# TheShinning/gps-sdr-sim

Hardware: AMD Instinct MI355X
Metric: IQ MSamples/s (and × real-time) at 2.6 MS/s, 12 sats, -b 16; 1/2/4/8 GPU (higher is better)
Workload: dtype int64 phases + f16 x f16 -> f32 MFMA accumulate (exact integer sums)

## Files before the change

### gps-sdr-sim_amd/csrc/common/gss_lin.h

```cpp
#ifndef GSS_LIN_H
#define GSS_LIN_H

#include <stdint.h>

#ifndef GSS_LIN_CH
#define GSS_LIN_CH     16
#endif
#define GSS_LIN_CHUNK  (64 * GSS_LIN_CH)
#define GSS_LIN_SEG    4096

#if defined(__HIPCC__)
#define GSS_LIN_FN static __host__ __device__ inline
#else
#define GSS_LIN_FN static inline
#endif

#define GSS_LIN_CSH    26

GSS_LIN_FN uint32_t gss_lin_dx(uint64_t xs) { return (uint32_t)((xs * 64u + (1ull << 31)) >> 32); }
GSS_LIN_FN uint32_t gss_lin_dz(uint64_t zs)
{
    return (uint32_t)((zs * 64u + (1ull << (GSS_LIN_CSH - 1))) >> GSS_LIN_CSH);
}
GSS_LIN_FN uint64_t gss_lin_xa(uint64_t xs)
// ... 50 lines not shown
}

typedef struct {
    uint64_t x;
    uint64_t z;
    int32_t g01;
    int32_t pos1;
    uint32_t npatch;
    uint32_t pad;
} gss_lin_row;
typedef struct {
    uint64_t xs, zs;
    uint64_t d;
    uint32_t dq;
    uint32_t tab;
} gss_lin_chan;

GSS_LIN_FN uint64_t gss_lin_mulhi(uint64_t a, uint64_t b)
{
#if defined(__HIP_DEVICE_COMPILE__)
    return __umul64hi(a, b);
#else
    return (uint64_t)(((unsigned __int128)a * b) >> 64);
#endif
}

GSS_LIN_FN uint64_t gss_lin_row_x(uint64_t x0, uint64_t xs, uint64_t n0)
{
    return x0 + n0 * xs + gss_lin_xa(xs);
}
GSS_LIN_FN uint64_t gss_lin_row_z(uint64_t z0, uint64_t zs, uint64_t n0)
{
    const uint64_t lo = z0 + n0 * zs;
    const uint64_t hi = gss_lin_mulhi(n0, zs) + (lo < z0 ? 1u : 0u);
    const uint32_t e0 = gss_lin_e0((hi << 14) | (lo >> 50));
    return (((uint64_t)e0 << 50) | (lo & ((1ull << 50) - 1))) + gss_lin_za(zs);
}
GSS_LIN_FN void gss_lin_row_gain(gss_lin_row *r, const int32_t *gpos, const int32_t *gval, int ngc,
                                 int32_t n0)
{
    int32_t g0 = gval[0], gn = 0, pn = INT32_MAX;
    for (int i = 1; i < ngc; i++) {
        const int32_t p = gpos[i], v = gval[i];
        g0 = p <= n0 ? v : g0;
    }
    for (int i = ngc - 1; i >= 1; i--) {
        const int32_t p = gpos[i], v = gval[i];
        gn = p > n0 ? v : gn;
        pn = p > n0 ? p : pn;
    }
    const int more = pn < n0 + GSS_LIN_SEG;
    const int32_t g1 = more ? gn : g0;
    r->g01 = (int32_t)(((uint32_t)g0 & 0xFFFFu) | ((uint32_t)g1 << 16));
    r->pos1 = more ? pn : INT32_MAX;
}
GSS_LIN_FN uint32_t gss_lin_row_npatch(const int32_t *ppos, int np, int32_t n0)
{
    uint32_t n = 0;
    for (int j = 0; j < np; j++)
        n += ppos[j] >= n0 && ppos[j] < n0 + GSS_LIN_SEG;
    return n;
}
GSS_LIN_FN gss_lin_row gss_lin_row_at(uint64_t x0, uint64_t xs, uint64_t z0, uint64_t zs,
                                      const int32_t *gpos, const int32_t *gval, int ngc,
                                      const int32_t *ppos, int np, int32_t n0)
{
    gss_lin_row r;
    r.x = gss_lin_row_x(x0, xs, (uint64_t)n0);
    r.z = gss_lin_row_z(z0, zs, (uint64_t)n0);
    gss_lin_row_gain(&r, gpos, gval, ngc, n0);
    r.npatch = gss_lin_row_npatch(ppos, np, n0);
    r.pad = 0;
    return r;
}
GSS_LIN_FN gss_lin_chan gss_lin_chan_of(uint64_t xs, uint64_t zs, uint32_t ca_tbl)
{
    gss_lin_chan c;
    c.xs = xs;
    c.zs = zs;
    c.d = ((uint64_t)gss_lin_dx(xs) << 32) | gss_lin_dz(zs);
    c.dq = (uint32_t)((zs * 64u) >> 46);
    c.tab = ca_tbl;
    return c;
}

typedef struct {
    int cell, chip;
} gss_lin_kc;

GSS_LIN_FN gss_lin_kc gss_lin_kernel_at(uint64_t x0, uint64_t xs, uint64_t z0, uint64_t zs,
                                         int64_t p)
{
    const int64_t c = p & ~(int64_t)(GSS_LIN_CHUNK - 1);
    const int64_t l = p & 63, s = (p - c) >> 6;
    const uint64_t lane = gss_lin_lane(xs, zs, (uint32_t)l);
    const int64_t n0 = p & ~(int64_t)(GSS_LIN_SEG - 1);
    const unsigned __int128 zn = (unsigned __int128)z0 + (unsigned __int128)(uint64_t)n0 * zs;
    const int64_t chips = (int64_t)(zn >> 50), e0 = gss_lin_e0((uint64_t)chips);
    const __int128 z = (__int128)z0 + (__int128)c * (__int128)zs -
                      (__int128)(chips - e0) * ((__int128)1 << 50);
    const unsigned __int128 zk = (unsigned __int128)((z + (int64_t)gss_lin_za(zs)) >> GSS_LIN_CSH);
    const uint64_t za = (uint64_t)(uint32_t)zk + (uint32_t)lane;
    const uint64_t zw = (uint64_t)(uint32_t)za + (uint64_t)s * gss_lin_dz(zs);
    const unsigned __int128 kz = zk + (uint32_t)lane + (unsigned __int128)(uint64_t)s *
                                 gss_lin_dz(zs);
    const uint32_t xb = (uint32_t)((x0 + (uint64_t)c * xs + gss_lin_xa(xs)) >> 32);
    const uint32_t xk = xb + (uint32_t)(lane >> 32) + (uint32_t)(za >> 32) +
                        (uint32_t)s * gss_lin_dx(xs) + (uint32_t)(zw >> 32);
    gss_lin_kc r;
    r.cell = (int)(xk >> 23);
    r.chip = (int)((uint64_t)(kz >> 24) % 1023u);
    return r;
}

#endif
```

### gps-sdr-sim_amd/csrc/hip/gss_synth.hip

```cpp
#include <hip/hip_runtime.h>
#include <stdint.h>
#include <stdlib.h>
#include <string.h>
#include "gpssim_amd.h"
#include "gss_dev.h"
#include "../common/gss_phase.h"
#include "../common/gss_lin.h"

#define SYNTH_THREADS  256
#define SYNTH_WAVES    (SYNTH_THREADS / 64)
#define ANCHOR_THREADS 64
#define CHUNK_BYTES    128
#define CHUNK_PIECES   (CHUNK_BYTES / 16)
#define LUT_N          1024

__global__ __launch_bounds__(ANCHOR_THREADS) void gss_anchor_kernel(
    const gss_chan_blk_t *__restrict__ blk, const int32_t *__restrict__ nch,
    const double *__restrict__ carr_ck, int nblk, int nchp, int n_per_blk, int nseg, int nsegp,
    int seg_r, double *__restrict__ seg_carr, double *__restrict__ seg_code,
    uint32_t *__restrict__ seg_cnt, double *__restrict__ carr_end,
    const int32_t *__restrict__ blist)
{
    const int nsub = carr_ck ? GSS_NCK : 1;
    const int nbw = (nblk + ANCHOR_THREADS - 1) / ANCHOR_THREADS;
// ... 298 lines not shown
                uint32_t ai = 64, aq = 64;
#pragma unroll
                for (int k = 0; k < NCH; k++) {
                    const int cv = (int)((uint32_t)e[k] << 10) >> 10;
                    const int sv = (e[k] - cv) >> 22;
                    ai += (uint32_t)g[k] * (uint32_t)cv;
                    aq += (uint32_t)g[k] * (uint32_t)sv;
                }
                acc_i = (int)ai;
                acc_q = (int)aq;
            }
#pragma unroll
            for (int k = 0; k < NCH; k++) {
                carr[k] = gss_carr_wrap(carr[k] + cs[k]);
                C[k] = C[k] + ks[k];
            }
            int i16 = (int)(int16_t)(acc_i >> 7);
            int q16 = (int)(int16_t)(acc_q >> 7);
            if (FMT == 16) {
                mine[sidx] = (uint32_t)(uint16_t)i16 | ((uint32_t)(uint16_t)q16 << 16);
            } else if (FMT == 8) {
                ((uint16_t *)mine)[sidx] = (uint16_t)((uint32_t)(uint8_t)(int8_t)(i16 >> 4) |
                                           ((uint32_t)(uint8_t)(int8_t)(q16 >> 4) << 8));
            } else {
                bits = (bits << 2) | ((uint32_t)(i16 > 0) << 1) | (uint32_t)(q16 > 0);
                if ((sidx & 15) == 15) {
                    int nb = nsamp - (sidx & ~15);
                    uint32_t w32 = nb >= 16 ? bits : nb > 0 ? (bits >> 2 * (16 - nb)) << 2 * (16 - nb) : 0u;
                    mine[sidx >> 4] = __builtin_bswap32(w32);
                    bits = 0;
                }
            }
        }
        if (last_seg && full && (ch + 1) * SPC == len) {
#pragma unroll
            for (int k = 0; k < NCH; k++) {
                const uint32_t c = s_st[k][tid];
                bad |= (C[k] >= GSS_CA_SEQ_LEN_D && c == (19u | (29u << 5) | (59u << 10))) ? 1 : 0;
            }
        }
        const bool any_full = __any(full);
        if (any_full) {
            wave_sync_lds();
            for (int i = 0; i < CHUNK_PIECES; i++) {
                int src = (64 / CHUNK_PIECES) * i + lane / CHUNK_PIECES, piece = lane % CHUNK_PIECES;
                int src_full = __shfl(full ? 1 : 0, src);
                if (src_full) {
                    uint8_t *sdst = dst + (ptrdiff_t)(src - lane) * ((ptrdiff_t)seg_r * BPS4 / 4) +
                                    (size_t)ch * CHUNK_BYTES + piece * 16;
                    const uint32_t *sp = stg + src * (CHUNK_BYTES / 4) + piece * 4;
                    store16(sdst, make_uint4(sp[0], sp[1], sp[2], sp[3]));
                }
            }
            wave_sync_lds();
        }
        if (!full && nsamp > 0) {
            int nbytes = nsamp * BPS4 / 4;
            uint8_t *bp = dst + (size_t)ch * CHUNK_BYTES;
            const uint8_t *sp = (const uint8_t *)mine;
            for (int i = 0; i < nbytes; i++)
                bp[i] = sp[i];
        }
    }
    if (bad && status)
        atomicOr(status, bad);
}

#define LIN_THREADS 256
#define LIN_WAVES   (LIN_THREADS / 64)
#define LIN_STEPS   (GSS_LIN_SEG / 64)
#define LIN_CH      GSS_LIN_CH
#define CBW_PRE     2
#define CBW_CHIPS   3072
#define CAB_W       ((CBW_CHIPS + 96) / 32)
static_assert(LIN_STEPS % LIN_CH == 0 && (LIN_CH & (LIN_CH - 1)) == 0, "whole chunks");
#define LIN_SW_SGPRS 68
typedef _Float16 lin_half4 __attribute__((ext_vector_type(4)));
typedef _Float16 lin_half8 __attribute__((ext_vector_type(8)));
typedef float lin_f4 __attribute__((ext_vector_type(4)));
#define LIN_GS    2
#define LIN_MAGF  (12582912.0f + 64.0f * LIN_GS)
#define LIN_MAGB  0x4B400000u

struct alignas(16) lin_ct {
    uint64_t B;
    uint64_t D;
    int32_t g;
    int32_t gd;
    int32_t pos1;
    uint32_t flags;
    uint32_t q0, dq, tab;
    uint32_t wa;
    uint32_t na, nb;
    uint32_t wn;
    uint32_t g2;
    uint32_t A[5][2];
};
static_assert(offsetof(lin_ct, A) % 8 == 0, "lin_ct.A: 8-byte reads");

typedef gss_lin_row lin_seg;
typedef gss_lin_chan lin_chan;
static_assert(sizeof(lin_seg) == 32 && sizeof(lin_chan) == 32, "two 16-byte LDS reads each");

__global__ void gss_cab_kernel(const uint32_t *__restrict__ ca_bits, int n_ca,
                               uint32_t *__restrict__ cab)
{
    const int i = blockIdx.x * blockDim.x + threadIdx.x;
    if (i >= n_ca * CAB_W)
        return;
    const int row = i / CAB_W, j0 = (i - row * CAB_W) * 32 - 32;
    const uint32_t *cb = ca_bits + (size_t)row * GSS_CA_WORDS;
    uint32_t w = 0;
    for (int q = 0; q < 32; q++) {
        const int e = j0 + q, chip = ((e % GSS_CA_LEN) + GSS_CA_LEN) % GSS_CA_LEN;
        w |= (((cb[chip >> 5] >> (chip & 31)) & 1u) ^ 1u) << q;
    }
    cab[i] = w;
}

__global__ void gss_tw16_kernel(const uint32_t *__restrict__ cab, int n_ca, uint32_t w,
                                uint32_t *__restrict__ tw)
{
    const int i = blockIdx.x * blockDim.x + threadIdx.x;
    if (i >= n_ca * GSS_LIN_TWE * LIN_CH)
        return;
    const int row = i / (GSS_LIN_TWE * LIN_CH), r = i - row * (GSS_LIN_TWE * LIN_CH);
    const int E = r / LIN_CH, st = r % LIN_CH;
    const uint32_t j = min((uint32_t)(E + (int)(((uint32_t)st * w) >> 4) - GSS_LIN_CBW_PRE + 32),
                           (uint32_t)(32 * CAB_W - 64));
    const uint32_t *c = cab + (size_t)row * CAB_W;
    const uint32_t lin = __builtin_amdgcn_alignbit(c[(j >> 5) + 1], c[j >> 5], j & 31);
    tw[i] = __builtin_amdgcn_alignbit(lin, lin, (32u - j) & 31u);
}

struct lin_wsrc {
    const uint32_t *W;
};

__device__ __forceinline__ void lin_wissue(const lin_wsrc &w, uint32_t (&ws)[LIN_CH])
{
#pragma unroll
    for (int s = 0; s < LIN_CH; s++)
        ws[s] = w.W[s];
}

__device__ __forceinline__ void lin_wfence(const uint32_t (&ws)[LIN_CH])
{
    static_assert(LIN_CH == 16, "the fence below names 16 windows");
    asm volatile("" :: "s"(ws[0]), "s"(ws[1]), "s"(ws[2]), "s"(ws[3]), "s"(ws[4]), "s"(ws[5]),
                 "s"(ws[6]), "s"(ws[7]), "s"(ws[8]), "s"(ws[9]), "s"(ws[10]), "s"(ws[11]),
                 "s"(ws[12]), "s"(ws[13]), "s"(ws[14]), "s"(ws[15]));
}

__device__ __forceinline__ lin_wsrc lin_wsrc_of(const lin_ct &t, const uint32_t *__restrict__ tw)
{
    const uint32_t off = __builtin_amdgcn_readfirstlane(t.wa);
    return lin_wsrc{(const uint32_t *)__builtin_assume_aligned(
        (const char *)tw + off, 64)};
}

#define LIN_SW_CLOBB "s84", "s85", "s86", "s87", "s88", "s89", "s90", "s91", "s92", "s93", "s94", \
                     "s95", "s96", "s97", "s98", "s99"
#define LIN_SW_CLOBA "s68", "s69", "s70", "s71", "s72", "s73", "s74", "s75", "s76", "s77", "s78", \
                     "s79", "s80", "s81", "s82", "s83"
#pragma clang diagnostic push
#pragma clang diagnostic ignored "-Winline-asm"
__device__ __forceinline__ void lin_sw_load(const uint32_t *__restrict__ tw, uint32_t off)
{
    const uint32_t *p = (const uint32_t *)((const char *)tw +
                                           (uint32_t)__builtin_amdgcn_readfirstlane(off));
    asm volatile("s_load_dwordx16 s[84:99], %0, 0x0" : : "s"(p) : LIN_SW_CLOBB);
}
__device__ __forceinline__ void lin_sw_load2(const uint32_t *__restrict__ tw, uint32_t off_a,
                                             uint32_t off_b)
{
    const uint32_t *pa = (const uint32_t *)((const char *)tw +
                                            (uint32_t)__builtin_amdgcn_readfirstlane(off_a));
    const uint32_t *pb = (const uint32_t *)((const char *)tw +
                                            (uint32_t)__builtin_amdgcn_readfirstlane(off_b));
    asm volatile("s_load_dwordx16 s[68:83], %0, 0x0\n\ts_load_dwordx16 s[84:99], %1, 0x0"
                 : : "s"(pa), "s"(pb) : LIN_SW_CLOBA, LIN_SW_CLOBB);
}
#pragma clang diagnostic pop
#define LIN_SW_TAKE(BUF, W)                                                                       \
    asm volatile("s_waitcnt lgkmcnt(0)\n\t"                                                      \
                 "s_mov_b64 %0, s[" #BUF "+0:" #BUF "+1]\n\ts_mov_b64 %1, s[" #BUF "+2:" #BUF "+3]\n\t" \
                 "s_mov_b64 %2, s[" #BUF "+4:" #BUF "+5]\n\ts_mov_b64 %3, s[" #BUF "+6:" #BUF "+7]\n\t" \
                 "s_mov_b64 %4, s[" #BUF "+8:" #BUF "+9]\n\ts_mov_b64 %5, s[" #BUF "+10:" #BUF "+11]\n\t" \
                 "s_mov_b64 %6, s[" #BUF "+12:" #BUF "+13]\n\ts_mov_b64 %7, s[" #BUF "+14:" #BUF "+15]" \
                 : "=s"(W[0]), "=s"(W[1]), "=s"(W[2]), "=s"(W[3]), "=s"(W[4]), "=s"(W[5]),      \
                   "=s"(W[6]), "=s"(W[7]))
__device__ __forceinline__ void lin_sw_split(const uint64_t (&w)[8], uint32_t (&ws)[LIN_CH])
{
    static_assert(LIN_CH == 16, "16 windows");
#pragma unroll
    for (int i = 0; i < 8; i++) {
        ws[2 * i] = (uint32_t)w[i];
        ws[2 * i + 1] = (uint32_t)(w[i] >> 32);
    }
}
__device__ __forceinline__ void lin_sw_take(uint32_t (&ws)[LIN_CH])
{
    uint64_t w[8];
    LIN_SW_TAKE(84, w);
    lin_sw_split(w, ws);
}
__device__ __forceinline__ void lin_sw_take_a(uint32_t (&ws)[LIN_CH])
{
    uint64_t w[8];
    LIN_SW_TAKE(68, w);
    lin_sw_split(w, ws);
}

template <bool LANE_GAIN, bool FIRST = false>
__device__ __forceinline__ void lin_channel_chunk_m(lin_f4 (&cq)[LIN_CH / 2], lin_f4 c0, uint64_t P,
                                                    uint64_t D, lin_wsrc W, uint32_t M,
                                                    lin_half4 A, int pos1, int p0,
                                                    const int32_t *__restrict__ s_lut)
{
    uint32_t e0 = 0;
    uint32_t sw[LIN_CH];
    lin_wissue(W, sw);
    lin_wfence(sw);
#pragma unroll
    for (int s = 0; s < LIN_CH; s++) {
        const uint32_t ws = sw[s];
        uint32_t t;
        asm("v_lshrrev_b32_sdwa %0, %1, %2 dst_sel:DWORD dst_unused:UNUSED_PAD src0_sel:BYTE_3 "
            "src1_sel:DWORD" : "=v"(t) : "v"((uint32_t)P), "s"(ws));
        const uint32_t a = __builtin_amdgcn_alignbit(t, (uint32_t)(P >> 32), 21) & M;
        uint32_t e = *(const uint32_t *)((const char *)s_lut + a);
        if (LANE_GAIN)
            e = p0 + s * 64 >= pos1 ? e : 0u;
        if (s & 1) {
            const uint2 bb = make_uint2(e0, e);
            cq[s / 2] = __builtin_amdgcn_mfma_f32_4x4x4f16(A, __builtin_bit_cast(lin_half4, bb),
                                                          FIRST ? c0 : cq[s / 2], 0, 0, 0);
        } else {
            e0 = e;
        }
        P += D;
    }
}

__device__ __forceinline__ void lin_sw_steps(lin_f4 (&cq)[LIN_CH / 2], const lin_ct &t, int k,
                                             int lane, const uint64_t *s_lane, uint32_t M,
                                             const int32_t *__restrict__ s_lut,
                                             const uint32_t (&ws)[LIN_CH])
{
    uint64_t P = s_lane[k * 64 + lane] + t.B;
    const uint64_t D = t.D;
    const lin_half4 A = __builtin_bit_cast(lin_half4, *(const uint2 *)t.A[lane & 3]);
    uint32_t e0 = 0;
#pragma unroll
    for (int s = 0; s < LIN_CH; s++) {
        uint32_t tt;
        asm("v_lshrrev_b32_sdwa %0, %1, %2 dst_sel:DWORD dst_unused:UNUSED_PAD src0_sel:BYTE_3 "
            "src1_sel:DWORD" : "=v"(tt) : "v"((uint32_t)P), "s"(ws[s]));
        const uint32_t a = __builtin_amdgcn_alignbit(tt, (uint32_t)(P >> 32), 21) & M;
        const uint32_t e = *(const uint32_t *)((const char *)s_lut + a);
        if (s & 1) {
            const uint2 bb = make_uint2(e0, e);
            cq[s / 2] = __builtin_amdgcn_mfma_f32_4x4x4f16(A, __builtin_bit_cast(lin_half4, bb),
                                                          cq[s / 2], 0, 0, 0);
        } else {
            e0 = e;
        }
        P += D;
    }
}

__device__ __forceinline__ uint32_t lin_pair_cls(int lane)
{
    const int q = lane >> 4, r = lane & 3;
    return ((lane & 15) >> 2) == q ? (uint32_t)r : 4u;
}

template <bool FIRST>
__device__ __forceinline__ void lin_sw_pair(lin_f4 (&cq)[LIN_CH / 2], lin_f4 c0, const lin_ct *T, int k0,
                                            int nc, int lane, const uint64_t *s_lane, uint32_t M,
                                            const int32_t *__restrict__ s_lut,
                                            const uint32_t *__restrict__ tw, uint32_t cls,
                                            bool more)
{
    const lin_ct &ta = T[k0], &tb = T[k0 + 1];
    uint64_t Pa = s_lane[k0 * 64 + lane] + ta.B, Pb = s_lane[(k0 + 1) * 64 + lane] + tb.B;
    const uint64_t Da = ta.D, Db = tb.D;
    const uint2 ga = *(const uint2 *)ta.A[cls], gb = *(const uint2 *)tb.A[cls];
    const lin_half8 A = __builtin_bit_cast(lin_half8, make_uint4(ga.x, ga.y, gb.x, gb.y));
    uint32_t na = ta.na, nb = ta.nb;
    asm volatile("" : "+v"(na), "+v"(nb));
    uint32_t wsa[LIN_CH], wsb[LIN_CH];
    lin_sw_take_a(wsa);
    lin_sw_take(wsb);
    if (k0 + 2 < nc || more)
        lin_sw_load2(tw, na, nb);
    uint32_t ea0 = 0, eb0 = 0;
#pragma unroll
    for (int s = 0; s < LIN_CH; s++) {
        uint32_t ta_, tb_;
        asm("v_lshrrev_b32_sdwa %0, %1, %2 dst_sel:DWORD dst_unused:UNUSED_PAD src0_sel:BYTE_3 "
            "src1_sel:DWORD" : "=v"(ta_) : "v"((uint32_t)Pa), "s"(wsa[s]));
        asm("v_lshrrev_b32_sdwa %0, %1, %2 dst_sel:DWORD dst_unused:UNUSED_PAD src0_sel:BYTE_3 "
            "src1_sel:DWORD" : "=v"(tb_) : "v"((uint32_t)Pb), "s"(wsb[s]));
        const uint32_t aa = __builtin_amdgcn_alignbit(ta_, (uint32_t)(Pa >> 32), 21) & M;
        const uint32_t ab = __builtin_amdgcn_alignbit(tb_, (uint32_t)(Pb >> 32), 21) & M;
        const uint32_t ea = *(const uint32_t *)((const char *)s_lut + aa);
        const uint32_t eb = *(const uint32_t *)((const char *)s_lut + ab);
        if (s & 1) {
            const uint4 bb = make_uint4(ea0, ea, eb0, eb);
            cq[s / 2] = __builtin_amdgcn_mfma_f32_16x16x32_f16(A, __builtin_bit_cast(lin_half8, bb),
                                                              FIRST ? c0 : cq[s / 2], 0, 0, 0);
        } else {
            ea0 = ea;
            eb0 = eb;
        }
        Pa += Da;
        Pb += Db;
    }
}

__device__ __forceinline__ lin_half4 lin_gain_operand(uint32_t gh, int lane)
{
    const uint32_t x = gh << ((lane & 1) * 16);
    const uint2 v = (lane & 2) ? make_uint2(0u, x) : make_uint2(x, 0u);
    return __builtin_bit_cast(lin_half4, v);
}

__host__ __device__ __forceinline__ uint32_t lin_f16_bits(int g)
{
    return (uint32_t)__builtin_bit_cast(uint16_t, (_Float16)(float)g);
}

__device__ __forceinline__ void lin_put(uint32_t *p, uint32_t v)
{
    __builtin_nontemporal_store(v, p);
}

extern "C" __device__ int gss_writelane(int, int, int) __asm("llvm.amdgcn.writelane.i32");

__device__ __forceinline__ uint32_t lin_ib(const lin_f4 (&cq)[LIN_CH / 2], int s)
{
    return __float_as_uint(cq[s / 2][2 * (s & 1)]);
}
__device__ __forceinline__ uint32_t lin_qb(const lin_f4 (&cq)[LIN_CH / 2], int s)
{
    return __float_as_uint(cq[s / 2][2 * (s & 1) + 1]);
}
__device__ __forceinline__ uint32_t lin_w16(const lin_f4 (&cq)[LIN_CH / 2], int s)
{
    const uint32_t pq = __builtin_amdgcn_perm(lin_qb(cq, s), lin_ib(cq, s), 0x06050201u);
    uint32_t r;
    asm("v_pk_add_u16 %0, %1, %2" : "=v"(r) : "v"(pq), "s"(0xC000C000u));
    return r;
}
__device__ __forceinline__ uint32_t lin_w8(const lin_f4 (&cq)[LIN_CH / 2], int s)
{
    constexpr uint32_t sh = 12u;
    uint32_t d = lin_ib(cq, s) >> sh;
    asm("v_lshrrev_b32_sdwa %0, %1, %2 dst_sel:BYTE_1 dst_unused:UNUSED_PRESERVE src0_sel:DWORD "
        "src1_sel:DWORD" : "+v"(d) : "v"(sh), "v"(lin_qb(cq, s)));
    return d;
}
__device__ __forceinline__ bool lin_ipos(const lin_f4 (&cq)[LIN_CH / 2], int s)
{
    return lin_ib(cq, s) >= LIN_MAGB + 128u * LIN_GS;
}
__device__ __forceinline__ bool lin_qpos(const lin_f4 (&cq)[LIN_CH / 2], int s)
{
    return lin_qb(cq, s) >= LIN_MAGB + 128u * LIN_GS;
}

template <int FMT, bool TAIL>
__device__ __forceinline__ void lin_store(const lin_f4 (&acc)[LIN_CH / 2], uint8_t *__restrict__ ob,
                                          int nb0, int lane, int n_per_blk)
{
    static_assert(FMT != 1 || LIN_CH == 16, "-b 1 packing assumes 16-step chunks");
    uint32_t pk[LIN_CH];
    pk[0] = 0;
#pragma unroll
    for (int s = 0; s < LIN_CH; s++) {
        const int nb = nb0 + s * 64, p = nb + lane;
        const bool in = !TAIL || p < n_per_blk;
        if (FMT == 16) {
            pk[s] = lin_w16(acc, s);
        } else if (FMT == 8) {
            const uint32_t v = lin_w8(acc, s);
            if (!TAIL)
                asm volatile("global_store_short %0, %1, %2 offset:%3"
                             : : "v"((uint32_t)lane * 2u), "v"(v),
                               "s"((uint16_t *)ob + nb0 + (s >> 4) * 2048), "i"((s & 15) * 128)
                             : "memory");
            else if (in)
                ((uint16_t *)ob)[p] = (uint16_t)v;
        } else {
            const uint64_t mi = __builtin_amdgcn_ballot_w64(lin_ipos(acc, s));
            const uint64_t mq = __builtin_amdgcn_ballot_w64(lin_qpos(acc, s));
            const uint32_t ilo = (uint32_t)mi, ihi = (uint32_t)(mi >> 32);
            const uint32_t qlo = (uint32_t)mq, qhi = (uint32_t)(mq >> 32);
            pk[0] = (uint32_t)gss_writelane((int)((ilo & 0xFFFFu) | (qlo << 16)), 4 * s, (int)pk[0]);
            pk[0] = (uint32_t)gss_writelane((int)((ilo >> 16) | (qlo & 0xFFFF0000u)), 4 * s + 1, (int)pk[0]);
            pk[0] = (uint32_t)gss_writelane((int)((ihi & 0xFFFFu) | (qhi << 16)), 4 * s + 2, (int)pk[0]);
            pk[0] = (uint32_t)gss_writelane((int)((ihi >> 16) | (qhi & 0xFFFF0000u)), 4 * s + 3, (int)pk[0]);
            (void)in;
        }
    }
    if (FMT == 1) {
        uint32_t vi = pk[0] & 0xFFFFu, vq = pk[0] >> 16;
        vi = (vi | (vi << 8)) & 0x00FF00FFu; vq = (vq | (vq << 8)) & 0x00FF00FFu;
        vi = (vi | (vi << 4)) & 0x0F0F0F0Fu; vq = (vq | (vq << 4)) & 0x0F0F0F0Fu;
        vi = (vi | (vi << 2)) & 0x33333333u; vq = (vq | (vq << 2)) & 0x33333333u;
        vi = (vi | (vi << 1)) & 0x55555555u; vq = (vq | (vq << 1)) & 0x55555555u;
        const uint32_t x = (vi << 1) | vq;
        const uint32_t y = ((x & 0x03030303u) << 6) | ((x & 0x0C0C0C0Cu) << 2) |
                           ((x >> 2) & 0x0C0C0C0Cu) | ((x >> 6) & 0x03030303u);
        uint8_t *dst = ob + nb0 / 4 + 4 * lane;
        const int first = nb0 + 16 * lane;
        const bool whole = !TAIL || first + 16 <= n_per_blk;
        if (whole && ((uintptr_t)(ob + nb0 / 4) & 3u) == 0) {
            lin_put((uint32_t *)dst, y);
        } else {
            for (int b = 0; b < 4; b++)
                if (first + 4 * b < n_per_blk)
                    dst[b] = (uint8_t)(y >> (8 * b));
        }
    }
    if (FMT == 16) {
        __builtin_amdgcn_sched_barrier(0);
        if (!TAIL) {
            uint32_t *base = (uint32_t *)ob + nb0;
            const uint32_t off = (uint32_t)lane * 4u;
#pragma unroll
            for (int s = 0; s < LIN_CH; s++)
                asm volatile("global_store_dword %0, %1, %2 offset:%3 nt"
                             : : "v"(off), "v"(pk[s]), "s"(base + (s >> 4) * 1024),
                               "i"((s & 15) * 256) : "memory");
        } else {
#pragma unroll
            for (int s = 0; s < LIN_CH; s++) {
                const int p = nb0 + s * 64 + lane;
                if (!TAIL || p < n_per_blk)
                    lin_put(((uint32_t *)ob) + p, pk[s]);
            }
        }
    }
}

__device__ __forceinline__ void lin_patch_fix(lin_f4 (&cq)[LIN_CH / 2],
                                              const gss_lin_t *__restrict__ Lk, int nb0, int lane)
{
    for (int j = 0; j < GSS_NPATCH; j++) {
        const int pp = Lk->ppos[j];
        if (pp >= nb0 + 64 * LIN_CH)
            break;
        if (pp < nb0)
            continue;
        const int q = pp - nb0;
        const int64_t d = lane == (q & 63) ? Lk->pdelta[j] : 0;
        const int di = (int)((uint32_t)d << 10) >> 10;
        const float fi = (float)(di * LIN_GS), fq = (float)((int)((d - di) >> 22) * LIN_GS);
        const int sq = __builtin_amdgcn_readfirstlane(q >> 6);
#pragma unroll
        for (int s = 0; s < LIN_CH; s++) {
            const float m = s == sq ? 1.0f : 0.0f;
            cq[s / 2][2 * (s & 1)] = __builtin_fmaf(m, fi, cq[s / 2][2 * (s & 1)]);
            cq[s / 2][2 * (s & 1) + 1] = __builtin_fmaf(m, fq, cq[s / 2][2 * (s & 1) + 1]);
        }
    }
}


#define LIN_MINB 4
template <int FMT>
__global__ __launch_bounds__(LIN_THREADS, LIN_MINB) __attribute__((amdgpu_num_sgpr(LIN_SW_SGPRS)))
void gss_lin_kernel(
    const gss_lin_t *__restrict__ lin, const gss_chan_blk_t *__restrict__ blk,
    const int32_t *__restrict__ nch, const int32_t *__restrict__ fast,
    const uint32_t *__restrict__ cab, const uint32_t *__restrict__ tw,
    const uint4 *__restrict__ lut16, int n_per_blk, int wg_per_blk,
    uint8_t *__restrict__ out, size_t block_bytes)
{
    __shared__ alignas(16) int32_t s_lut[1024];
    __shared__ uint64_t s_lane[GSS_MAXCH * 64];
    __shared__ lin_ct s_ct[LIN_WAVES][GSS_MAXCH];
    __shared__ alignas(16) lin_seg s_seg[LIN_WAVES][GSS_MAXCH];
    __shared__ alignas(16) lin_chan s_chan[GSS_MAXCH];
    const int b = blockIdx.x / wg_per_blk;
    const int w = blockIdx.x - b * wg_per_blk;
    if (!fast[b])
        return;
    const int tid = threadIdx.x, lane = tid & 63;
    const int wave = __builtin_amdgcn_readfirstlane(tid >> 6);
    static_assert(sizeof(s_lut) == LIN_THREADS * sizeof(uint4), "one 16-byte copy per thread");
    const uint4 lutv = lut16[tid];
    const gss_lin_t *L = lin + (size_t)b * GSS_MAXCH;
    const int nc = nch[b];
#pragma unroll
    for (int j = 0; j < GSS_MAXCH / LIN_WAVES; j++) {
        const int k = wave + j * LIN_WAVES;
        if (k < nc)
            s_lane[k * 64 + lane] = gss_lin_lane(L[k].xs, L[k].zs, (uint32_t)lane);
    }
    {
        const int rk = lane & (GSS_MAXCH - 1), rj = lane / GSS_MAXCH;
        static_assert(LIN_WAVES * GSS_MAXCH == 64 && LIN_WAVES == 4, "one row per lane, 4 parts");
        const int rn0 = (w * LIN_WAVES + rj) * (64 * LIN_STEPS);
        if (rk < nc && rn0 < n_per_blk) {
            const gss_lin_t *Lk = L + rk;
            lin_seg &r = s_seg[rj][rk];
            if (wave == 0) {
                r.x = gss_lin_row_x(Lk->x0, Lk->xs, (uint64_t)rn0);
                r.z = gss_lin_row_z(Lk->z0, Lk->zs, (uint64_t)rn0);
            } else if (wave == 1) {
                gss_lin_row g;
                gss_lin_row_gain(&g, Lk->gpos, Lk->gval, GSS_NGC, rn0);
                r.g01 = g.g01;
                r.pos1 = g.pos1;
            } else if (wave == 2) {
                r.npatch = gss_lin_row_npatch(Lk->ppos, GSS_NPATCH, rn0);
                r.pad = 0;
            } else if (rj == 0) {
                s_chan[rk] = gss_lin_chan_of(Lk->xs, Lk->zs,
                                             (uint32_t)blk[(size_t)b * GSS_MAXCH + rk].ca_tbl);
            }
        }
    }
    ((uint4 *)s_lut)[tid] = lutv;
    (void)cab;
    __syncthreads();
    uint32_t M = 0xFFCu;
    asm volatile("" : "+v"(M));
    const uint32_t cls = lin_pair_cls(lane);
    lin_f4 c0 = lin_f4{LIN_MAGF, LIN_MAGF, LIN_MAGF, LIN_MAGF};
    asm volatile("" : "+v"(c0));
    const int sg = w * LIN_WAVES + wave;
    const int n0 = sg * (64 * LIN_STEPS);
    if (n0 >= n_per_blk)
        return;
    lin_ct *T = s_ct[wave];
    uint8_t *ob = out + (size_t)b * block_bytes;
    bool sw_ahead = false;
    uint64_t xb = 0, zb = 0, xs10 = 0, zs10 = 0;
    int32_t pos1 = INT32_MAX;
    uint32_t pflag = 0, gh0 = 0, gh1 = 0;
    uint32_t trow = 0, wa_next = 0;
    int g_after = -1;
    if (lane < nc) {
        const lin_chan ck = s_chan[lane];
        const lin_seg sk = s_seg[wave][lane];
        xb = sk.x;
        zb = sk.z;
        xs10 = ck.xs << 10;
        zs10 = ck.zs << 10;
        static_assert(64 * LIN_CH == 1024, "one chunk = 2^10 samples");
        pos1 = sk.pos1;
        pflag = sk.npatch != 0 ? 2u : 0u;
        const int g0 = (int)(int16_t)(sk.g01 & 0xFFFF), g1 = sk.g01 >> 16;
        gh0 = lin_f16_bits(g0 * LIN_GS);
        gh1 = lin_f16_bits(g1 * LIN_GS);
        lin_ct &t = T[lane];
        t.D = ck.d;
        t.gd = g1 - g0;
        t.pos1 = sk.pos1;
        t.dq = ck.dq;
        t.tab = ck.tab;
        t.A[4][0] = 0;
        t.A[4][1] = 0;
        trow = ck.tab * GSS_LIN_TWE;
        wa_next = (trow + min((uint32_t)(zb >> 50), (uint32_t)(GSS_LIN_TWE - 1))) *
                  (uint32_t)(LIN_CH * sizeof(uint32_t));
    }

    const int nc_blk = nc;
    for (int c = 0; c < LIN_STEPS / LIN_CH; c++) {
        int nc = nc_blk;
        asm volatile("" : "+s"(nc));
        const int nb0 = n0 + c * (64 * LIN_CH);
        if (nb0 >= n_per_blk)
            break;
        const bool after = pos1 <= nb0;
        const bool chg = pos1 < nb0 + 64 * LIN_CH;
        const uint32_t my_flags = (chg && !after ? 1u : 0u) | pflag;
        const uint64_t zn = zb + zs10;
        const uint32_t my_wa = wa_next;
        const uint32_t my_wn = (trow + min((uint32_t)(zn >> 50), (uint32_t)(GSS_LIN_TWE - 1))) *
                               (uint32_t)(LIN_CH * sizeof(uint32_t));
        if (lane < nc) {
            lin_ct &t = T[lane];
            t.B = (xb & ~0xFFFFFFFFull) | (uint32_t)(zb >> GSS_LIN_CSH);
            t.flags = my_flags;
            t.wa = my_wa;
            t.wn = my_wn;
            if ((int)after != g_after) {
                g_after = (int)after;
                const uint32_t gh = after ? gh1 : gh0;
                t.A[0][0] = gh;         t.A[0][1] = 0;
                t.A[1][0] = gh << 16;   t.A[1][1] = 0;
                t.A[2][0] = 0;          t.A[2][1] = gh;
                t.A[3][0] = 0;          t.A[3][1] = gh << 16;
                t.g2 = gh | (gh << 16);
            }
        }
        wa_next = my_wn;
        xb += xs10;
        zb = zn;
        const uint32_t wa0 = (uint32_t)__builtin_amdgcn_readlane((int)my_wa, 0);
        const uint32_t wa1r = (uint32_t)__builtin_amdgcn_readlane((int)my_wa, 1);
        const uint32_t wn0 = (uint32_t)__builtin_amdgcn_readlane((int)my_wn, 0);
        const uint32_t wn1r = (uint32_t)__builtin_amdgcn_readlane((int)my_wn, 1);
        const uint32_t wa1 = nc > 1 ? wa1r : wa0, wn1 = nc > 1 ? wn1r : wn0;
        {
            const uint32_t wa2 = (uint32_t)__builtin_amdgcn_update_dpp(0, (int)my_wa, 0x102, 0xF,
                                                                       0xF, true);
            const uint32_t wa3 = (uint32_t)__builtin_amdgcn_update_dpp(0, (int)my_wa, 0x103, 0xF,
                                                                       0xF, true);
            if (lane < nc) {
                const bool in2 = lane + 2 < nc, in3 = lane + 3 < nc;
                T[lane].na = in2 ? wa2 : wn0;
                T[lane].nb = in3 ? wa3 : in2 ? wa2 : wn1;
            }
        }
        const uint64_t fmask = __builtin_amdgcn_ballot_w64(my_flags != 0);
        wave_sync_lds();
        lin_f4 acc[LIN_CH / 2];
        if (nc > 0 && !sw_ahead)
            lin_sw_load2(tw, wa0, wa1);
        const bool more = c + 1 < LIN_STEPS / LIN_CH && nb0 + 64 * LIN_CH < n_per_blk;
        int k0 = 0;
        if (nc >= 2) {
            lin_sw_pair<true>(acc, c0, T, 0, nc, lane, s_lane, M, s_lut, tw, cls, more);
            k0 = 2;
        } else {
#pragma unroll
            for (int s = 0; s < LIN_CH / 2; s++) {
                lin_f4 v = c0;
                asm volatile("" : "+v"(v));
                acc[s] = v;
            }
        }
#pragma unroll
        for (int p = 1; p < GSS_MAXCH / 2; p++) {
            if (2 * p + 1 >= nc)
                break;
            lin_sw_pair<false>(acc, c0, T, 2 * p, nc, lane, s_lane, M, s_lut, tw, cls, more);
            k0 = 2 * p + 2;
        }
        if (k0 < nc) {
            uint32_t ws[LIN_CH], wb[LIN_CH];
            lin_sw_take_a(ws);
            lin_sw_take(wb);
            (void)wb;
            if (more)
                lin_sw_load2(tw, wn0, wn1);
            lin_sw_steps(acc, T[k0], k0, lane, s_lane, M, s_lut, ws);
            k0 = nc;
        }
        sw_ahead = nc > 0 && more;
        for (int k = k0; k < nc; k++) {
            const lin_ct &t = T[k];
            const uint64_t B = t.B, D = t.D;
            const uint2 a2 = *(const uint2 *)t.A[lane & 3];
            lin_channel_chunk_m<false>(acc, c0, s_lane[k * 64 + lane] + B, D, lin_wsrc_of(t, tw), M,
                                       __builtin_bit_cast(lin_half4, a2), 0, 0, s_lut);
        }
        for (uint64_t fm = fmask; fm; fm &= fm - 1) {
            const int k = __builtin_amdgcn_readfirstlane((int)__builtin_ctzll(fm));
            const lin_ct &t = T[k];
            const uint64_t B = t.B, D = t.D;
            const uint32_t fl = __builtin_amdgcn_readfirstlane(t.flags);
            if (__builtin_expect(fl & 1u, 0)) {
                uint32_t l2 = (uint32_t)lane;
                asm volatile("" : "+v"(l2));
                lin_channel_chunk_m<true>(acc, c0, s_lane[k * 64 + l2] + B, D, lin_wsrc_of(t, tw), M,
                                          lin_gain_operand(lin_f16_bits(t.gd * LIN_GS), (int)l2), t.pos1,
                                          nb0 + (int)l2, s_lut);
            }
            if (__builtin_expect(fl & 2u, 0))
                lin_patch_fix(acc, L + k, nb0, lane);
        }
        wave_sync_lds();
        if (nb0 + 64 * LIN_CH <= n_per_blk)
            lin_store<FMT, false>(acc, ob, nb0, lane, n_per_blk);
        else
            lin_store<FMT, true>(acc, ob, nb0, lane, n_per_blk);
    }
}


#define GSS_STR2(x) #x
#define GSS_STR(x) GSS_STR2(x)
extern "C" int gss_dev_ordinal(const gss_dev *d) { return d->ordinal; }

extern "C" const char *gss_build_info(void)
{
    return "lin_mfma=2 lin_ch=" GSS_STR(LIN_CH) " lin_swin=3 spec_k=" GSS_STR(GSS_SPEC_K)
           " arch=gfx950";
}


extern "C" void gss_run_pool_prewarm(int dev);
extern "C" void gss_run_pool_drain(int dev);

struct host_tables {
    gss_dev_tables dev;
    lut_arg lut;
};

static const host_tables &tables_once()
{
    static const host_tables made = [] {
        host_tables h;
        int32_t s[512], c[512];
        gss_lut(s, c);
        for (int i = 0; i < 512; i++) {
            h.lut.sin512[i] = h.dev.lut[512 + i] = (int16_t)s[i];
            h.lut.cos512[i] = h.dev.lut[i] = (int16_t)c[i];
            const uint32_t v = lin_f16_bits(c[i]) | (lin_f16_bits(s[i]) << 16);
            h.dev.lut16[i] = v;
            h.dev.lut16[512 + i] = v ^ 0x80008000u;
        }
        gss_ca_table(h.dev.ca);
        gss_noise_table(h.dev.noise);
        return h;
    }();
    return made;
}

static int dev_init(gss_dev *d)
{
    const char *r = getenv("GSS_SEG_R");
    if (r && atoi(r) >= 256 && atoi(r) % 256 == 0)
        d->seg_r = atoi(r);
    for (int i = 0; i < gss_dev::RING; i++)
        for (int j = 0; j < 2; j++) {
            HIP_TRY(hipEventCreate(&d->ev_a[i][j]));
            HIP_TRY(hipEventCreate(&d->ev_b[i][j]));
            HIP_TRY(hipEventCreate(&d->ev_l[i][j]));
        }
    const host_tables &h = tables_once();
    d->lut = h.lut;
    int rc = d->tab.reserve(sizeof h.dev, "constant tables");
    if (rc == 0) rc = d->d_status.reserve(sizeof(int32_t), "render status");
    if (rc) return rc;
    HIP_TRY(hipMemcpy(d->tab.p, &h.dev, sizeof h.dev, hipMemcpyHostToDevice));
    int prio_lo = 0, prio_hi = 0;
    HIP_TRY(hipDeviceGetStreamPriorityRange(&prio_lo, &prio_hi));
    HIP_TRY(hipStreamCreateWithPriority(&d->aux, hipStreamNonBlocking, prio_hi));
    HIP_TRY(hipEventCreateWithFlags(&d->ev_in, hipEventDisableTiming));
    HIP_TRY(hipEventCreateWithFlags(&d->ev_fb, hipEventDisableTiming));
    gss_run_pool_prewarm(d->ordinal);
    return 0;
}

extern "C" int gss_dev_open(gss_dev **out, int ordinal)
{
    *out = nullptr;
    int count = 0;
    if (hipGetDeviceCount(&count) != hipSuccess || count <= 0)
        return gss_fail(GSS_E_NODEV, "no HIP device visible");
    if (ordinal < 0 || ordinal >= count)
        return gss_fail(GSS_E_ARG, "device ordinal %d out of range (%d devices)", ordinal, count);
    HIP_TRY(hipSetDevice(ordinal));
    gss_dev *d = new gss_dev();
// ... 438 lines not shown
```

Measured before the change: 509,100.

## Precompute all per-chunk channel records up front, one lane per (chunk, channel)

Builds the per-(chunk, channel) records (B, table-row offsets, flags, gain operands) for every chunk of a wave's segment in one pass before the chunk loop. Each of the 64 lanes handles one (chunk, channel) pair, and the next-window offsets come from ds_bpermute. This removes the per-chunk LDS record update, the readlane/DPP shuffles and the two wave_sync_lds barriers from the inner loop, and lets pair loads read B, D and the gain operand as 16-byte vectors. In exchange it uses more shared memory per wave, adds an up-front setup cost, and relies on LIN_CHUNKS*GSS_MAXCH being exactly 64.

```diff
diff --git a/gps-sdr-sim_amd/csrc/common/gss_lin.h b/gps-sdr-sim_amd/csrc/common/gss_lin.h
--- a/gps-sdr-sim_amd/csrc/common/gss_lin.h
+++ b/gps-sdr-sim_amd/csrc/common/gss_lin.h
@@ -156,6 +156,37 @@
     c.dq = (uint32_t)((zs * 64u) >> 46);
     c.tab = ca_tbl;
     return c;
+}
+
+#define GSS_LIN_REC_GAIN  1u
+#define GSS_LIN_REC_PATCH 2u
+typedef struct {
+    uint64_t B;
+    uint32_t wa, wn;
+    uint32_t flags;
+    int32_t g;
+} gss_lin_chunk;
+
+GSS_LIN_FN uint32_t gss_lin_wrow(uint32_t tab, uint64_t zb)
+{
+    const uint32_t e = (uint32_t)(zb >> 50);
+    return (tab * GSS_LIN_TWE + (e < GSS_LIN_TWE - 1u ? e : GSS_LIN_TWE - 1u)) *
+           (uint32_t)(GSS_LIN_CH * sizeof(uint32_t));
+}
+GSS_LIN_FN void gss_lin_chunk_rec(const gss_lin_row *row, const gss_lin_chan *chan, int32_t n0,
+                                  int c, gss_lin_chunk *rec)
+{
+    const uint64_t xc = chan->xs * (uint64_t)GSS_LIN_CHUNK, zc = chan->zs * (uint64_t)GSS_LIN_CHUNK;
+    const uint64_t xb = row->x + ((c & 1) ? xc : 0u) + ((c & 2) ? xc << 1 : 0u);
+    const uint64_t zb = row->z + ((c & 1) ? zc : 0u) + ((c & 2) ? zc << 1 : 0u);
+    const int32_t nb0 = n0 + c * GSS_LIN_CHUNK;
+    const int after = row->pos1 <= nb0;
+    const int inside = !after && row->pos1 < nb0 + GSS_LIN_CHUNK;
+    rec->B = (xb & ~0xFFFFFFFFull) | (uint32_t)(zb >> GSS_LIN_CSH);
+    rec->wa = gss_lin_wrow(chan->tab, zb);
+    rec->wn = gss_lin_wrow(chan->tab, zb + zc);
+    rec->flags = (inside ? GSS_LIN_REC_GAIN : 0u) | (row->npatch != 0 ? GSS_LIN_REC_PATCH : 0u);
+    rec->g = after ? row->g01 >> 16 : (int32_t)(int16_t)(row->g01 & 0xFFFF);
 }
 
 typedef struct {
diff --git a/gps-sdr-sim_amd/csrc/hip/gss_synth.hip b/gps-sdr-sim_amd/csrc/hip/gss_synth.hip
--- a/gps-sdr-sim_amd/csrc/hip/gss_synth.hip
+++ b/gps-sdr-sim_amd/csrc/hip/gss_synth.hip
@@ -404,21 +404,21 @@
 #define LIN_MAGF  (12582912.0f + 64.0f * LIN_GS)
 #define LIN_MAGB  0x4B400000u
 
-struct alignas(16) lin_ct {
-    uint64_t B;
-    uint64_t D;
-    int32_t g;
-    int32_t gd;
-    int32_t pos1;
-    uint32_t flags;
-    uint32_t q0, dq, tab;
-    uint32_t wa;
-    uint32_t na, nb;
-    uint32_t wn;
-    uint32_t g2;
-    uint32_t A[5][2];
+#define LIN_CHUNKS (LIN_STEPS / LIN_CH)
+struct alignas(16) lin_ck {
+    uint64_t B[GSS_MAXCH];
+    uint32_t A[GSS_MAXCH / 2][5][4];
 };
-static_assert(offsetof(lin_ct, A) % 8 == 0, "lin_ct.A: 8-byte reads");
+struct alignas(16) lin_wrec {
+    uint64_t D[GSS_MAXCH];
+    int32_t gd[GSS_MAXCH];
+    int32_t pos1[GSS_MAXCH];
+    lin_ck ck[LIN_CHUNKS];
+};
+static_assert(LIN_CHUNKS * GSS_MAXCH == 64, "one lane per (chunk, channel) record");
+static_assert(offsetof(lin_wrec, D) % 16 == 0 && offsetof(lin_wrec, ck) % 16 == 0 &&
+              offsetof(lin_ck, B) % 16 == 0 && offsetof(lin_ck, A) % 16 == 0 &&
+              sizeof(lin_ck) % 16 == 0, "16-byte reads of a pair's B, D and gain operand");
 
 typedef gss_lin_row lin_seg;
 typedef gss_lin_chan lin_chan;
@@ -474,9 +474,9 @@
                  "s"(ws[12]), "s"(ws[13]), "s"(ws[14]), "s"(ws[15]));
 }
 
-__device__ __forceinline__ lin_wsrc lin_wsrc_of(const lin_ct &t, const uint32_t *__restrict__ tw)
-{
-    const uint32_t off = __builtin_amdgcn_readfirstlane(t.wa);
+__device__ __forceinline__ lin_wsrc lin_wsrc_of(uint32_t wa, const uint32_t *__restrict__ tw)
+{
+    const uint32_t off = __builtin_amdgcn_readfirstlane(wa);
     return lin_wsrc{(const uint32_t *)__builtin_assume_aligned(
         (const char *)tw + off, 64)};
 }
@@ -544,6 +544,7 @@
     uint32_t sw[LIN_CH];
     lin_wissue(W, sw);
     lin_wfence(sw);
+    const int first = pos1 - p0;
 #pragma unroll
     for (int s = 0; s < LIN_CH; s++) {
         const uint32_t ws = sw[s];
@@ -553,7 +554,7 @@
         const uint32_t a = __builtin_amdgcn_alignbit(t, (uint32_t)(P >> 32), 21) & M;
         uint32_t e = *(const uint32_t *)((const char *)s_lut + a);
         if (LANE_GAIN)
-            e = p0 + s * 64 >= pos1 ? e : 0u;
+            e = s * 64 >= first ? e : 0u;
         if (s & 1) {
             const uint2 bb = make_uint2(e0, e);
             cq[s / 2] = __builtin_amdgcn_mfma_f32_4x4x4f16(A, __builtin_bit_cast(lin_half4, bb),
@@ -565,14 +566,15 @@
     }
 }
 
-__device__ __forceinline__ void lin_sw_steps(lin_f4 (&cq)[LIN_CH / 2], const lin_ct &t, int k,
-                                             int lane, const uint64_t *s_lane, uint32_t M,
+__device__ __forceinline__ void lin_sw_steps(lin_f4 (&cq)[LIN_CH / 2], const lin_wrec *R,
+                                             const lin_ck *T, int k, int lane,
+                                             const uint64_t *s_lane, uint32_t M,
                                              const int32_t *__restrict__ s_lut,
                                              const uint32_t (&ws)[LIN_CH])
 {
-    uint64_t P = s_lane[k * 64 + lane] + t.B;
-    const uint64_t D = t.D;
-    const lin_half4 A = __builtin_bit_cast(lin_half4, *(const uint2 *)t.A[lane & 3]);
+    uint64_t P = s_lane[k * 64 + lane] + T->B[k];
+    const uint64_t D = R->D[k];
+    const lin_half4 A = __builtin_bit_cast(lin_half4, *(const uint2 *)T->A[k / 2][lane & 3]);
     uint32_t e0 = 0;
 #pragma unroll
     for (int s = 0; s < LIN_CH; s++) {
@@ -599,24 +601,24 @@
 }
 
 template <bool FIRST>
-__device__ __forceinline__ void lin_sw_pair(lin_f4 (&cq)[LIN_CH / 2], lin_f4 c0, const lin_ct *T, int k0,
-                                            int nc, int lane, const uint64_t *s_lane, uint32_t M,
+__device__ __forceinline__ void lin_sw_pair(lin_f4 (&cq)[LIN_CH / 2], lin_f4 c0, const lin_wrec *R,
+                                            const lin_ck *T, int k0, int lane,
+                                            const uint64_t *s_lane, uint32_t M,
                                             const int32_t *__restrict__ s_lut,
                                             const uint32_t *__restrict__ tw, uint32_t cls,
-                                            bool more)
-{
-    const lin_ct &ta = T[k0], &tb = T[k0 + 1];
-    uint64_t Pa = s_lane[k0 * 64 + lane] + ta.B, Pb = s_lane[(k0 + 1) * 64 + lane] + tb.B;
-    const uint64_t Da = ta.D, Db = tb.D;
-    const uint2 ga = *(const uint2 *)ta.A[cls], gb = *(const uint2 *)tb.A[cls];
-    const lin_half8 A = __builtin_bit_cast(lin_half8, make_uint4(ga.x, ga.y, gb.x, gb.y));
-    uint32_t na = ta.na, nb = ta.nb;
-    asm volatile("" : "+v"(na), "+v"(nb));
+                                            uint32_t na, uint32_t nb, int la, bool load)
+{
+    const uint4 B2 = *(const uint4 *)&T->B[k0], D2 = *(const uint4 *)&R->D[k0];
+    uint64_t Pa = s_lane[k0 * 64 + lane] + (((uint64_t)B2.y << 32) | B2.x);
+    uint64_t Pb = s_lane[(k0 + 1) * 64 + lane] + (((uint64_t)B2.w << 32) | B2.z);
+    const uint64_t Da = ((uint64_t)D2.y << 32) | D2.x, Db = ((uint64_t)D2.w << 32) | D2.z;
+    const lin_half8 A = __builtin_bit_cast(lin_half8, *(const uint4 *)T->A[k0 / 2][cls]);
     uint32_t wsa[LIN_CH], wsb[LIN_CH];
     lin_sw_take_a(wsa);
     lin_sw_take(wsb);
-    if (k0 + 2 < nc || more)
-        lin_sw_load2(tw, na, nb);
+    if (load)
+        lin_sw_load2(tw, (uint32_t)__builtin_amdgcn_readlane((int)na, la),
+                     (uint32_t)__builtin_amdgcn_readlane((int)nb, la));
     uint32_t ea0 = 0, eb0 = 0;
 #pragma unroll
     for (int s = 0; s < LIN_CH; s++) {
@@ -645,7 +647,8 @@
 __device__ __forceinline__ lin_half4 lin_gain_operand(uint32_t gh, int lane)
 {
     const uint32_t x = gh << ((lane & 1) * 16);
-    const uint2 v = (lane & 2) ? make_uint2(0u, x) : make_uint2(x, 0u);
+    const uint32_t hi = x & (uint32_t)-((lane >> 1) & 1);
+    const uint2 v = make_uint2(x ^ hi, hi);
     return __builtin_bit_cast(lin_half4, v);
 }
 
@@ -804,7 +807,7 @@
 {
     __shared__ alignas(16) int32_t s_lut[1024];
     __shared__ uint64_t s_lane[GSS_MAXCH * 64];
-    __shared__ lin_ct s_ct[LIN_WAVES][GSS_MAXCH];
+    __shared__ lin_wrec s_rec[LIN_WAVES];
     __shared__ alignas(16) lin_seg s_seg[LIN_WAVES][GSS_MAXCH];
     __shared__ alignas(16) lin_chan s_chan[GSS_MAXCH];
     const int b = blockIdx.x / wg_per_blk;
@@ -859,98 +862,64 @@
     const int n0 = sg * (64 * LIN_STEPS);
     if (n0 >= n_per_blk)
         return;
-    lin_ct *T = s_ct[wave];
+    const lin_wrec *R = &s_rec[wave];
     uint8_t *ob = out + (size_t)b * block_bytes;
-    bool sw_ahead = false;
-    uint64_t xb = 0, zb = 0, xs10 = 0, zs10 = 0;
-    int32_t pos1 = INT32_MAX;
-    uint32_t pflag = 0, gh0 = 0, gh1 = 0;
-    uint32_t trow = 0, wa_next = 0;
-    int g_after = -1;
-    if (lane < nc) {
-        const lin_chan ck = s_chan[lane];
-        const lin_seg sk = s_seg[wave][lane];
-        xb = sk.x;
-        zb = sk.z;
-        xs10 = ck.xs << 10;
-        zs10 = ck.zs << 10;
-        static_assert(64 * LIN_CH == 1024, "one chunk = 2^10 samples");
-        pos1 = sk.pos1;
-        pflag = sk.npatch != 0 ? 2u : 0u;
-        const int g0 = (int)(int16_t)(sk.g01 & 0xFFFF), g1 = sk.g01 >> 16;
-        gh0 = lin_f16_bits(g0 * LIN_GS);
-        gh1 = lin_f16_bits(g1 * LIN_GS);
-        lin_ct &t = T[lane];
-        t.D = ck.d;
-        t.gd = g1 - g0;
-        t.pos1 = sk.pos1;
-        t.dq = ck.dq;
-        t.tab = ck.tab;
-        t.A[4][0] = 0;
-        t.A[4][1] = 0;
-        trow = ck.tab * GSS_LIN_TWE;
-        wa_next = (trow + min((uint32_t)(zb >> 50), (uint32_t)(GSS_LIN_TWE - 1))) *
-                  (uint32_t)(LIN_CH * sizeof(uint32_t));
-    }
+    uint32_t my_wa = 0, my_flags = 0;
+    const int pk = lane & (GSS_MAXCH - 1), pc = lane / GSS_MAXCH;
+    if (pk < nc) {
+        const lin_chan ck = s_chan[pk];
+        const lin_seg sk = s_seg[wave][pk];
+        gss_lin_chunk r;
+        gss_lin_chunk_rec(&sk, &ck, n0, pc, &r);
+        my_wa = r.wa;
+        my_flags = r.flags;
+        lin_wrec &wr = s_rec[wave];
+        lin_ck &t = wr.ck[pc];
+        t.B[pk] = r.B;
+        const uint32_t gh = lin_f16_bits(r.g * LIN_GS);
+        uint32_t (&A)[5][4] = t.A[pk / 2];
+        const int h = 2 * (pk & 1);
+        *(uint2 *)&A[0][h] = make_uint2(gh, 0u);
+        *(uint2 *)&A[1][h] = make_uint2(gh << 16, 0u);
+        *(uint2 *)&A[2][h] = make_uint2(0u, gh);
+        *(uint2 *)&A[3][h] = make_uint2(0u, gh << 16);
+        *(uint2 *)&A[4][h] = make_uint2(0u, 0u);
+        if (pc == 0) {
+            wr.D[pk] = ck.d;
+            wr.gd[pk] = (sk.g01 >> 16) - (int)(int16_t)(sk.g01 & 0xFFFF);
+            wr.pos1[pk] = sk.pos1;
+        }
+    }
+    uint32_t my_na, my_nb;
+    {
+        const bool in2 = pk + 2 < nc, in3 = pk + 3 < nc;
+        const int nxt = (pc * GSS_MAXCH + GSS_MAXCH) & 63;
+        const int sa = in2 ? lane + 2 : nxt;
+        const int sb = in3 ? lane + 3 : in2 ? lane + 2 : nxt + (nc > 1 ? 1 : 0);
+        my_na = (uint32_t)__builtin_amdgcn_ds_bpermute(sa << 2, (int)my_wa);
+        my_nb = (uint32_t)__builtin_amdgcn_ds_bpermute(sb << 2, (int)my_wa);
+    }
+    const uint64_t fmask = __builtin_amdgcn_ballot_w64(my_flags != 0);
+    wave_sync_lds();
+    if (nc > 0)
+        lin_sw_load2(tw, (uint32_t)__builtin_amdgcn_readlane((int)my_wa, 0),
+                     (uint32_t)__builtin_amdgcn_readlane((int)my_wa, nc > 1 ? 1 : 0));
 
     const int nc_blk = nc;
-    for (int c = 0; c < LIN_STEPS / LIN_CH; c++) {
+    for (int c = 0; c < LIN_CHUNKS; c++) {
         int nc = nc_blk;
         asm volatile("" : "+s"(nc));
         const int nb0 = n0 + c * (64 * LIN_CH);
         if (nb0 >= n_per_blk)
             break;
-        const bool after = pos1 <= nb0;
-        const bool chg = pos1 < nb0 + 64 * LIN_CH;
-        const uint32_t my_flags = (chg && !after ? 1u : 0u) | pflag;
-        const uint64_t zn = zb + zs10;
-        const uint32_t my_wa = wa_next;
-        const uint32_t my_wn = (trow + min((uint32_t)(zn >> 50), (uint32_t)(GSS_LIN_TWE - 1))) *
-                               (uint32_t)(LIN_CH * sizeof(uint32_t));
-        if (lane < nc) {
-            lin_ct &t = T[lane];
-            t.B = (xb & ~0xFFFFFFFFull) | (uint32_t)(zb >> GSS_LIN_CSH);
-            t.flags = my_flags;
-            t.wa = my_wa;
-            t.wn = my_wn;
-            if ((int)after != g_after) {
-                g_after = (int)after;
-                const uint32_t gh = after ? gh1 : gh0;
-                t.A[0][0] = gh;         t.A[0][1] = 0;
-                t.A[1][0] = gh << 16;   t.A[1][1] = 0;
-                t.A[2][0] = 0;          t.A[2][1] = gh;
-                t.A[3][0] = 0;          t.A[3][1] = gh << 16;
-                t.g2 = gh | (gh << 16);
-            }
-        }
-        wa_next = my_wn;
-        xb += xs10;
-        zb = zn;
-        const uint32_t wa0 = (uint32_t)__builtin_amdgcn_readlane((int)my_wa, 0);
-        const uint32_t wa1r = (uint32_t)__builtin_amdgcn_readlane((int)my_wa, 1);
-        const uint32_t wn0 = (uint32_t)__builtin_amdgcn_readlane((int)my_wn, 0);
-        const uint32_t wn1r = (uint32_t)__builtin_amdgcn_readlane((int)my_wn, 1);
-        const uint32_t wa1 = nc > 1 ? wa1r : wa0, wn1 = nc > 1 ? wn1r : wn0;
-        {
-            const uint32_t wa2 = (uint32_t)__builtin_amdgcn_update_dpp(0, (int)my_wa, 0x102, 0xF,
-                                                                       0xF, true);
-            const uint32_t wa3 = (uint32_t)__builtin_amdgcn_update_dpp(0, (int)my_wa, 0x103, 0xF,
-                                                                       0xF, true);
-            if (lane < nc) {
-                const bool in2 = lane + 2 < nc, in3 = lane + 3 < nc;
-                T[lane].na = in2 ? wa2 : wn0;
-                T[lane].nb = in3 ? wa3 : in2 ? wa2 : wn1;
-            }
-        }
-        const uint64_t fmask = __builtin_amdgcn_ballot_w64(my_flags != 0);
-        wave_sync_lds();
+        const lin_ck *T = &R->ck[c];
+        const int l0 = c * GSS_MAXCH;
         lin_f4 acc[LIN_CH / 2];
-        if (nc > 0 && !sw_ahead)
-            lin_sw_load2(tw, wa0, wa1);
-        const bool more = c + 1 < LIN_STEPS / LIN_CH && nb0 + 64 * LIN_CH < n_per_blk;
+        const bool more = c + 1 < LIN_CHUNKS && nb0 + 64 * LIN_CH < n_per_blk;
         int k0 = 0;
         if (nc >= 2) {
-            lin_sw_pair<true>(acc, c0, T, 0, nc, lane, s_lane, M, s_lut, tw, cls, more);
+            lin_sw_pair<true>(acc, c0, R, T, 0, lane, s_lane, M, s_lut, tw, cls, my_na, my_nb, l0,
+                              2 < nc || more);
             k0 = 2;
         } else {
 #pragma unroll
@@ -964,7 +933,8 @@
         for (int p = 1; p < GSS_MAXCH / 2; p++) {
             if (2 * p + 1 >= nc)
                 break;
-            lin_sw_pair<false>(acc, c0, T, 2 * p, nc, lane, s_lane, M, s_lut, tw, cls, more);
+            lin_sw_pair<false>(acc, c0, R, T, 2 * p, lane, s_lane, M, s_lut, tw, cls, my_na, my_nb,
+                               l0 + 2 * p, 2 * p + 2 < nc || more);
             k0 = 2 * p + 2;
         }
         if (k0 < nc) {
@@ -973,34 +943,25 @@
             lin_sw_take(wb);
             (void)wb;
             if (more)
-                lin_sw_load2(tw, wn0, wn1);
-            lin_sw_steps(acc, T[k0], k0, lane, s_lane, M, s_lut, ws);
-            k0 = nc;
-        }
-        sw_ahead = nc > 0 && more;
-        for (int k = k0; k < nc; k++) {
-            const lin_ct &t = T[k];
-            const uint64_t B = t.B, D = t.D;
-            const uint2 a2 = *(const uint2 *)t.A[lane & 3];
-            lin_channel_chunk_m<false>(acc, c0, s_lane[k * 64 + lane] + B, D, lin_wsrc_of(t, tw), M,
-                                       __builtin_bit_cast(lin_half4, a2), 0, 0, s_lut);
-        }
-        for (uint64_t fm = fmask; fm; fm &= fm - 1) {
-            const int k = __builtin_amdgcn_readfirstlane((int)__builtin_ctzll(fm));
-            const lin_ct &t = T[k];
-            const uint64_t B = t.B, D = t.D;
-            const uint32_t fl = __builtin_amdgcn_readfirstlane(t.flags);
-            if (__builtin_expect(fl & 1u, 0)) {
+                lin_sw_load2(tw, (uint32_t)__builtin_amdgcn_readlane((int)my_na, l0 + k0),
+                             (uint32_t)__builtin_amdgcn_readlane((int)my_nb, l0 + k0));
+            lin_sw_steps(acc, R, T, k0, lane, s_lane, M, s_lut, ws);
+        }
+        for (uint32_t fm = (uint32_t)(fmask >> l0) & ((1u << GSS_MAXCH) - 1u); fm; fm &= fm - 1) {
+            const int k = __builtin_amdgcn_readfirstlane(__builtin_ctz(fm));
+            const uint32_t fl = (uint32_t)__builtin_amdgcn_readlane((int)my_flags, l0 + k);
+            if (__builtin_expect(fl & GSS_LIN_REC_GAIN, 0)) {
+                const uint32_t wa = (uint32_t)__builtin_amdgcn_readlane((int)my_wa, l0 + k);
                 uint32_t l2 = (uint32_t)lane;
                 asm volatile("" : "+v"(l2));
-                lin_channel_chunk_m<true>(acc, c0, s_lane[k * 64 + l2] + B, D, lin_wsrc_of(t, tw), M,
-                                          lin_gain_operand(lin_f16_bits(t.gd * LIN_GS), (int)l2), t.pos1,
-                                          nb0 + (int)l2, s_lut);
+                lin_channel_chunk_m<true>(acc, c0, s_lane[k * 64 + l2] + T->B[k], R->D[k],
+                                          lin_wsrc_of(wa, tw), M,
+                                          lin_gain_operand(lin_f16_bits(R->gd[k] * LIN_GS), (int)l2),
+                                          R->pos1[k], nb0 + (int)l2, s_lut);
             }
-            if (__builtin_expect(fl & 2u, 0))
+            if (__builtin_expect(fl & GSS_LIN_REC_PATCH, 0))
                 lin_patch_fix(acc, L + k, nb0, lane);
         }
-        wave_sync_lds();
         if (nb0 + 64 * LIN_CH <= n_per_blk)
             lin_store<FMT, false>(acc, ob, nb0, lane, n_per_blk);
         else
```

New measurement: 517,400 (median of 6 runs). 1.6% higher.
